# microsoft/tf2-gnn

Hardware: AMD Instinct MI355X
Metric: edges/sec (fwd+bwd) RGCN H=320 L=4, PPI-shaped batch, 1/2/4/8 MI355X (higher is better)
Workload: dtype f32; 1 GPU; rmat30k: V=30000 E=900000 per GPU (one batch per rank, replicas) edge_types=4 D=320 H=320 layers=4 RGCN (PPI_RGCN.json stack settings), step = edge bucketing of the next batch (2nd stream, overlapped) + forward (training mode) + f...

## Files before the change

### tf2_gnn_amd/csrc/graph.hip

```cpp
#include <algorithm>
#include <cstdlib>
#include <mutex>
#include <vector>

#include "common.hpp"
#include "graph.hpp"

namespace tfgnn {

static thread_local char g_err[512] = "";

void set_error(const char* fmt, ...) {
  va_list ap;
  va_start(ap, fmt);
  vsnprintf(g_err, sizeof(g_err), fmt, ap);
  va_end(ap);
}

static int64_t g_launch_counts[TFGNN_KFAM_COUNT] = {0};
void count_launch(int family) {
  if (family >= 0 && family < TFGNN_KFAM_COUNT) __atomic_fetch_add(&g_launch_counts[family], 1, __ATOMIC_RELAXED);
}

}
// ... 53 lines not shown
  for (int w = 0; w < (tid >> 6); ++w) wave_off += wave_tot[w];
  int32_t excl = wave_off + incl - sum;
#pragma unroll
  for (int i = 0; i < SCAN_ITEMS; ++i) {
    int64_t idx = base + i;
    if (idx < n) out[idx] = excl;
    excl += v[i];
  }
  if (tid == SCAN_THREADS - 1 && block_sums) block_sums[blockIdx.x] = wave_off + incl;
}

__global__ void __launch_bounds__(SCAN_THREADS)
scan_add_offsets_kernel(int32_t* __restrict__ out, const int32_t* __restrict__ block_offs, int64_t n) {
  const int32_t off = block_offs[blockIdx.x];
  const int64_t base = (int64_t)blockIdx.x * SCAN_TILE;
  for (int i = threadIdx.x; i < SCAN_TILE; i += SCAN_THREADS) {
    int64_t idx = base + i;
    if (idx < n) out[idx] += off;
  }
}

static size_t scan_scratch_elems(int64_t n) {
  size_t total = 0;
  while (n > SCAN_TILE) {
    n = ceil_div(n, SCAN_TILE);
    total += (size_t)n;
  }
  return total + 1;
}

static int exclusive_scan_i32(const int32_t* in, int32_t* out, int64_t n, int32_t* scratch,
                              hipStream_t s) {
  if (n <= 0) return TFGNN_OK;
  int64_t nb = ceil_div(n, SCAN_TILE);
  if (nb == 1) {
    hipLaunchKernelGGL(scan_tiles_kernel, dim3(1), dim3(SCAN_THREADS), 0, s, in, out, (int32_t*)nullptr, n);
    TFGNN_LAUNCH_CHECK();
    return TFGNN_OK;
  }
  hipLaunchKernelGGL(scan_tiles_kernel, dim3((unsigned)nb), dim3(SCAN_THREADS), 0, s, in, out, scratch, n);
  TFGNN_LAUNCH_CHECK();
  int rc = exclusive_scan_i32(scratch, scratch, nb, scratch + nb, s);
  if (rc) return rc;
  hipLaunchKernelGGL(scan_add_offsets_kernel, dim3((unsigned)nb), dim3(SCAN_THREADS), 0, s, out, scratch, n);
  TFGNN_LAUNCH_CHECK();
  return TFGNN_OK;
}

constexpr int EL_INLINE = 8;
struct EdgeLists {
  const int32_t* const* adj;
  const int64_t* edge_off;
  const int32_t* adj_v[EL_INLINE];
  int64_t off_v[EL_INLINE + 1];
  int L;
  int inline_tables;
};

__device__ __forceinline__ int find_type(const int64_t* __restrict__ edge_off, int L, int64_t g) {
  int lo = 0, hi = L;
  while (hi - lo > 1) {
    int mid = (lo + hi) >> 1;
    if (edge_off[mid] <= g) lo = mid; else hi = mid;
  }
  return lo;
}

__device__ __forceinline__ void load_edge(const EdgeLists& el, int64_t g, int64_t& src, int64_t& dst, int& l) {
  const int32_t* a;
  if (el.inline_tables) {
    l = 0;
#pragma unroll
    for (int i = 1; i < EL_INLINE; ++i) l += (i < el.L && el.off_v[i] <= g) ? 1 : 0;
    a = el.adj_v[l] + 2 * (g - el.off_v[l]);
  } else {
    l = find_type(el.edge_off, el.L, g);
    a = el.adj[l] + 2 * (g - el.edge_off[l]);
  }
  src = a[0];
  dst = a[1];
}

constexpr int RS_THREADS = 512;
constexpr int RS_ROUNDS = 16;
constexpr int RS_WAVES = RS_THREADS / 64;
constexpr int RS_WAVE_KEYS = 64 * RS_ROUNDS;
constexpr int RS_TILE = RS_THREADS * RS_ROUNDS;
constexpr int RS_DIGIT_BITS = 9;
constexpr int RS_RADIX = 1 << RS_DIGIT_BITS;
static_assert(RS_RADIX == RS_THREADS, "one digit per thread");

template <typename KeyT>
__global__ void __launch_bounds__(RS_THREADS)
fill_keys_kernel(EdgeLists el, int64_t E, int64_t V, int sec_bits, KeyT* __restrict__ comp_d, KeyT* __restrict__ comp_s,
                 int32_t* __restrict__ hist, int nblk_ld, int32_t* __restrict__ err_flag) {
  __shared__ int32_t h[2][RS_RADIX];
  const int tid = threadIdx.x;
  h[0][tid] = 0;
  h[1][tid] = 0;
  __syncthreads();
  const int64_t base = (int64_t)blockIdx.x * RS_TILE;
#pragma unroll 4
  for (int r = 0; r < RS_ROUNDS; ++r) {
    const int64_t g = base + r * RS_THREADS + tid;
    if (g < E) {
      int64_t src, dst;
      int l;
      load_edge(el, g, src, dst, l);
      if (src < 0 || src >= V || dst < 0 || dst >= V) {
        atomicOr(err_flag, 1);
        src = 0;
        dst = 0;
      }
      const KeyT kd = (KeyT)(((uint64_t)(dst * el.L + l) << sec_bits) | (uint64_t)src);
      const KeyT ks = (KeyT)(((uint64_t)(src * el.L + l) << sec_bits) | (uint64_t)dst);
      comp_d[g] = kd;
      comp_s[g] = ks;
      atomicAdd(&h[0][(int)((kd >> sec_bits) & (RS_RADIX - 1))], 1);
      atomicAdd(&h[1][(int)((ks >> sec_bits) & (RS_RADIX - 1))], 1);
    }
  }
  __syncthreads();
  hist[(int64_t)tid * nblk_ld + blockIdx.x] = h[0][tid];
  hist[(int64_t)(RS_RADIX + tid) * nblk_ld + blockIdx.x] = h[1][tid];
}

template <typename KeyT>
__global__ void __launch_bounds__(RS_THREADS)
rs_hist_kernel(const KeyT* __restrict__ comp_d, const KeyT* __restrict__ comp_s, int64_t n, int shift,
               int32_t* __restrict__ hist, int nblk_ld) {
  __shared__ int32_t h[RS_RADIX];
  const int tid = threadIdx.x;
  const int side = blockIdx.y;
  const KeyT* __restrict__ comp = side ? comp_s : comp_d;
  h[tid] = 0;
  __syncthreads();
  const int64_t base = (int64_t)blockIdx.x * RS_TILE;
#pragma unroll 4
  for (int r = 0; r < RS_ROUNDS; ++r) {
    const int64_t idx = base + r * RS_THREADS + tid;
    if (idx < n) atomicAdd(&h[(int)((comp[idx] >> shift) & (RS_RADIX - 1))], 1);
  }
  __syncthreads();
  hist[(int64_t)(side * RS_RADIX + tid) * nblk_ld + blockIdx.x] = h[tid];
}

template <typename KeyT, bool PAY>
__global__ void __launch_bounds__(RS_THREADS)
rs_scatter_kernel(const KeyT* __restrict__ in_d, const KeyT* __restrict__ in_s, const uint32_t* __restrict__ pin_d,
                  const uint32_t* __restrict__ pin_s, int64_t n, int shift, const int32_t* __restrict__ hist, int nblk,
                  int nblk_ld, KeyT* __restrict__ out_d, KeyT* __restrict__ out_s, uint32_t* __restrict__ pout_d,
                  uint32_t* __restrict__ pout_s) {
  __shared__ int32_t wbase[RS_WAVES][RS_RADIX];
  __shared__ int32_t wtot[RS_WAVES];
  const int tid = threadIdx.x;
  const int lane = tid & 63, wave = tid >> 6;
  const int side = blockIdx.y;
  const KeyT* __restrict__ kin = side ? in_s : in_d;
  const uint32_t* __restrict__ pin = side ? pin_s : pin_d;
  KeyT* __restrict__ kout = side ? out_s : out_d;
  uint32_t* __restrict__ pout = side ? pout_s : pout_d;
  volatile int32_t* mine_base = &wbase[wave][0];
#pragma unroll
  for (int i = 0; i < RS_RADIX / 64; ++i) mine_base[lane + 64 * i] = 0;
  __builtin_amdgcn_wave_barrier();
  const int64_t wave0 = (int64_t)blockIdx.x * RS_TILE + (int64_t)wave * RS_WAVE_KEYS;
  const unsigned long long lt_mask = lane == 0 ? 0ull : (~0ull >> (64 - lane));
  KeyT key[RS_ROUNDS];
  uint32_t pl[PAY ? RS_ROUNDS : 1];
  int32_t info[RS_ROUNDS];
#pragma unroll
  for (int r = 0; r < RS_ROUNDS; ++r) {
    const int64_t idx = wave0 + r * 64 + lane;
    const bool valid = idx < n;
    key[r] = valid ? kin[idx] : (KeyT)0;
    if (PAY) pl[r] = valid ? (pin ? pin[idx] : (uint32_t)idx) : 0u;
  }
#pragma unroll
  for (int r = 0; r < RS_ROUNDS; ++r) {
    const bool valid = wave0 + r * 64 + lane < n;
    const int d = (int)((key[r] >> shift) & (RS_RADIX - 1));
    unsigned long long peers = __ballot(valid);
#pragma unroll
    for (int b = 0; b < RS_DIGIT_BITS; ++b) {
      const unsigned long long m = __ballot((d >> b) & 1);
      peers &= ((d >> b) & 1) ? m : ~m;
    }
    const int rank = __popcll(peers & lt_mask);
    const int cnt = __popcll(peers);
    info[r] = valid ? (rank | (cnt << 8) | (1 << 16)) : 0;
    if (valid && rank == 0) mine_base[d] = mine_base[d] + cnt;
    __builtin_amdgcn_wave_barrier();
  }
  __syncthreads();
  int32_t tot = 0, before = 0;
  {
    const int32_t* __restrict__ row = hist + (int64_t)(side * RS_RADIX + tid) * nblk_ld;
    const int me = (int)blockIdx.x;
    for (int b0 = 0; b0 < nblk; b0 += 16) {
      int4 v[4];
#pragma unroll
      for (int u = 0; u < 4; ++u)
        v[u] = b0 + 4 * u < nblk ? *reinterpret_cast<const int4*>(row + b0 + 4 * u) : make_int4(0, 0, 0, 0);
#pragma unroll
      for (int u = 0; u < 4; ++u) {
        const int b = b0 + 4 * u;
        const int e[4] = {v[u].x, v[u].y, v[u].z, v[u].w};
#pragma unroll
        for (int k = 0; k < 4; ++k)
          if (b + k < nblk) {
            tot += e[k];
            if (b + k < me) before += e[k];
          }
      }
    }
  }
  int32_t incl = tot;
#pragma unroll
  for (int o = 1; o < 64; o <<= 1) {
    const int32_t t = __shfl_up(incl, o, 64);
    if (lane >= o) incl += t;
  }
  if (lane == 63) wtot[wave] = incl;
  __syncthreads();
  {
    int32_t off = 0;
    for (int w = 0; w < wave; ++w) off += wtot[w];
    int32_t running = off + incl - tot + before;
#pragma unroll
    for (int w = 0; w < RS_WAVES; ++w) {
      const int32_t c = wbase[w][tid];
      wbase[w][tid] = running;
      running += c;
    }
  }
  __syncthreads();
#pragma unroll
  for (int r = 0; r < RS_ROUNDS; ++r) {
    const bool valid = (info[r] >> 16) & 1;
    const int d = (int)((key[r] >> shift) & (RS_RADIX - 1));
    const int rank = info[r] & 255, cnt = (info[r] >> 8) & 255;
    const int32_t b = valid ? mine_base[d] : 0;
    __builtin_amdgcn_wave_barrier();
    if (valid && rank == 0) mine_base[d] = b + cnt;
    __builtin_amdgcn_wave_barrier();
    if (valid) {
      kout[b + rank] = key[r];
      if (PAY) pout[b + rank] = pl[r];
    }
  }
}

template <typename KeyT>
__global__ void rowptr_from_sorted_kernel(const KeyT* __restrict__ comp_d, const KeyT* __restrict__ comp_s, int64_t E,
                                          int sec_bits, int64_t R, int32_t* __restrict__ rowptr_d,
                                          int32_t* __restrict__ rowptr_s) {
  const KeyT* __restrict__ comp = blockIdx.y ? comp_s : comp_d;
  int32_t* __restrict__ rowptr = blockIdx.y ? rowptr_s : rowptr_d;
  for (int64_t r = (int64_t)blockIdx.x * blockDim.x + threadIdx.x; r <= R; r += (int64_t)gridDim.x * blockDim.x) {
    int64_t lo = 0, hi = E;
    while (lo < hi) {
      const int64_t mid = (lo + hi) >> 1;
      if ((int64_t)((uint64_t)comp[mid] >> sec_bits) < r) lo = mid + 1; else hi = mid;
    }
    rowptr[r] = (int32_t)lo;
  }
}

struct PlanJob {
  const int32_t* rowptr;
  int64_t R;
  int thr, chunk;
  int32_t* counters;
  int32_t *item_row, *item_chunk, *item_slot, *multi_row, *multi_base, *multi_n;
  int32_t *bin_count, *bin_cursor, *short_rows;
  int want_items;
};
struct PlanJobs {
  PlanJob j[2];
};

__device__ __forceinline__ void plan_rows_body(const int32_t* __restrict__ rowptr, int64_t R, int long_threshold, int chunk_edges,
                                 int32_t* __restrict__ counters,
                                 int32_t* __restrict__ item_row, int32_t* __restrict__ item_chunk,
                                 int32_t* __restrict__ item_slot, int32_t* __restrict__ multi_row,
                                 int32_t* __restrict__ multi_base, int32_t* __restrict__ multi_n) {
  for (int64_t r = (int64_t)blockIdx.x * blockDim.x + threadIdx.x; r < R; r += (int64_t)gridDim.x * blockDim.x) {
    const int32_t len = rowptr[r + 1] - rowptr[r];
    if (len <= long_threshold) continue;
    const int32_t n = (len + chunk_edges - 1) / chunk_edges;
    const int32_t base = atomicAdd(&counters[0], n);
    int32_t pb = -1;
    if (n > 1) {
      const int32_t m = atomicAdd(&counters[1], 1);
      pb = atomicAdd(&counters[2], n);
      multi_row[m] = (int32_t)r;
      multi_base[m] = pb;
      multi_n[m] = n;
// ... 58 lines not shown
      acc += bin_count[i];
    }
  }
  constexpr int TILE = 256 * SHORT_TILE_ROWS;
  for (int64_t tile = blockIdx.x; tile * TILE < R; tile += gridDim.x) {
    for (int i = threadIdx.x; i <= thr; i += 256) h[i] = 0;
    __syncthreads();
    int32_t len[SHORT_TILE_ROWS];
    int rank[SHORT_TILE_ROWS];
#pragma unroll
    for (int k = 0; k < SHORT_TILE_ROWS; ++k) {
      const int64_t r = tile * TILE + k * 256 + threadIdx.x;
      len[k] = r < R ? rowptr[r + 1] - rowptr[r] : -1;
      rank[k] = (len[k] >= 0 && len[k] <= thr) ? atomicAdd(&h[len[k]], 1) : 0;
    }
    __syncthreads();
    for (int i = threadIdx.x; i <= thr; i += 256)
      if (h[i]) base[i] = atomicAdd(&bin_cursor[i], h[i]);
    __syncthreads();
#pragma unroll
    for (int k = 0; k < SHORT_TILE_ROWS; ++k)
      if (len[k] >= 0 && len[k] <= thr)
        short_rows[start[len[k]] + base[len[k]] + rank[k]] = (int32_t)(tile * TILE + k * 256 + threadIdx.x);
    __syncthreads();
  }
}

__global__ void nz_flags_kernel(const int32_t* __restrict__ rowptr, int64_t V, int L, int32_t* __restrict__ flags,
                                int32_t* __restrict__ node_cnt) {
  const int64_t R = V * L;
  for (int64_t i = (int64_t)blockIdx.x * blockDim.x + threadIdx.x; i <= R; i += (int64_t)gridDim.x * blockDim.x) {
    if (i < R) {
      const int64_t l = i / V, v = i - l * V;
      const int64_t r = v * L + l;
      flags[i] = rowptr[r + 1] > rowptr[r] ? 1 : 0;
    } else {
      flags[i] = 0;
    }
    if (i <= V) {
      int32_t c = 0;
      if (i < V)
        for (int l = 0; l < L; ++l) c += rowptr[i * L + l + 1] > rowptr[i * L + l] ? 1 : 0;
      node_cnt[i] = c;
    }
  }
}

__global__ void nz_fill_kernel(const int32_t* __restrict__ rowptr, const int32_t* __restrict__ scan_t, int64_t V,
                               int L, int32_t* __restrict__ cpos, int32_t* __restrict__ nzrow,
                               int32_t* __restrict__ nz_node, int32_t* __restrict__ nz_off) {
  const int64_t R = V * L;
  for (int64_t i = (int64_t)blockIdx.x * blockDim.x + threadIdx.x; i < R; i += (int64_t)gridDim.x * blockDim.x) {
    const int64_t l = i / V, v = i - l * V;
    const int64_t r = v * L + l;
    const int32_t c = scan_t[i];
    if (rowptr[r + 1] > rowptr[r]) {
      cpos[r] = c;
      nzrow[c] = (int32_t)r;
      nz_node[c] = (int32_t)v;
    } else {
      cpos[r] = -1;
    }
    if (v == 0) nz_off[l] = c;
    if (i == R - 1) nz_off[L] = scan_t[R];
  }
}

__global__ void nz_cols_kernel(const int32_t* __restrict__ cpos, const int32_t* __restrict__ nodeptr_nz, int64_t V,
                               int L, int32_t* __restrict__ col_nz) {
  for (int64_t v = (int64_t)blockIdx.x * blockDim.x + threadIdx.x; v < V; v += (int64_t)gridDim.x * blockDim.x) {
    int32_t j = nodeptr_nz[v];
    for (int l = 0; l < L; ++l) {
      const int32_t c = cpos[v * L + l];
      if (c >= 0) col_nz[j++] = c;
    }
  }
}

__device__ __forceinline__ int node_pattern(const int32_t* __restrict__ rowptr, int64_t v, int L) {
  int m = 0;
  for (int l = 0; l < L; ++l) m |= (rowptr[v * L + l + 1] > rowptr[v * L + l]) ? (1 << l) : 0;
  return m;
}
__global__ void __launch_bounds__(256) pattern_count_kernel(const int32_t* __restrict__ rowptr, int64_t V, int L,
                                                            int32_t* __restrict__ bins ) {
  __shared__ int h[256];
  h[threadIdx.x] = 0;
  __syncthreads();
  for (int64_t v = (int64_t)blockIdx.x * 256 + threadIdx.x; v < V; v += (int64_t)gridDim.x * 256) atomicAdd(&h[node_pattern(rowptr, v, L)], 1);
  __syncthreads();
  if (h[threadIdx.x]) atomicAdd(&bins[threadIdx.x], h[threadIdx.x]);
}
__global__ void __launch_bounds__(256) pattern_place_kernel(const int32_t* __restrict__ rowptr, int64_t V, int L,
                                                            const int32_t* __restrict__ bins, int32_t* __restrict__ cursor ,
                                                            int32_t* __restrict__ pos, int32_t* __restrict__ node_at,
                                                            int32_t* __restrict__ rowmap) {
  __shared__ int base[256], h[256], slot0[256];
  {
    h[threadIdx.x] = bins[threadIdx.x];
    __syncthreads();
    const int key = ((8 - __popc((int)threadIdx.x)) << 8) | (int)threadIdx.x;
    int acc = 0;
    for (int m = 0; m < 256; ++m) acc += ((((8 - __popc(m)) << 8) | m) < key) ? h[m] : 0;
    base[threadIdx.x] = acc;
    __syncthreads();
  }
  for (int64_t v0 = (int64_t)blockIdx.x * 256; v0 < V; v0 += (int64_t)gridDim.x * 256) {
    h[threadIdx.x] = 0;
    __syncthreads();
    const int64_t v = v0 + threadIdx.x;
    int m = 0, rank = 0;
    if (v < V) {
      m = node_pattern(rowptr, v, L);
      rank = atomicAdd(&h[m], 1);
    }
    __syncthreads();
    if (h[threadIdx.x]) slot0[threadIdx.x] = atomicAdd(&cursor[threadIdx.x], h[threadIdx.x]);
    __syncthreads();
    if (v < V) {
      const int32_t p = base[m] + slot0[m] + rank;
      if (pos) pos[v] = p;
      node_at[p] = (int32_t)v;
      if (rowmap)
        for (int l = 0; l < L; ++l) rowmap[v * L + l] = p * L + l;
    }
    __syncthreads();
  }
}
__global__ void __launch_bounds__(128) pattern_tilemask_kernel(const int32_t* __restrict__ rowptr, const int32_t* __restrict__ node_at,
                                                               int64_t V, int L, uint8_t* __restrict__ tilemask) {
  __shared__ int m;
  if (threadIdx.x == 0) m = 0;
  __syncthreads();
  const int64_t p = (int64_t)blockIdx.x * 128 + threadIdx.x;
  if (p < V) atomicOr(&m, node_pattern(rowptr, node_at[p], L));
  __syncthreads();
  if (threadIdx.x == 0) tilemask[blockIdx.x] = (uint8_t)m;
}

template <typename KeyT, bool PAY>
__global__ void unpack_kernel(const KeyT* __restrict__ comp_d, const KeyT* __restrict__ comp_s, const uint32_t* __restrict__ pay_d,
                              const uint32_t* __restrict__ pay_s, int sec_bits, int64_t E, int L, int64_t R,
                              const int32_t* __restrict__ rowptr_d, const int32_t* __restrict__ rowptr_s,
                              int32_t* __restrict__ col_d, int32_t* __restrict__ eid_d, int32_t* __restrict__ coll_d,
                              float* __restrict__ invdeg_edge_d, int32_t* __restrict__ eid_to_pos, int32_t* __restrict__ row_node,
                              int32_t* __restrict__ col_s, int32_t* __restrict__ eid_s, int32_t* __restrict__ coll_s,
                              float* __restrict__ invdeg_edge_s, float* __restrict__ invdeg_d, int32_t* __restrict__ nodeptr_d,
                              int32_t* __restrict__ nodeptr_s, int first_job) {
  const int job = (int)blockIdx.y + first_job;
  if (job == 2) {
    for (int64_t r = (int64_t)blockIdx.x * blockDim.x + threadIdx.x; r <= R; r += (int64_t)gridDim.x * blockDim.x) {
      if (r < R) {
        const int32_t len = rowptr_d[r + 1] - rowptr_d[r];
        invdeg_d[r] = len > 0 ? 1.0f / ((float)len + kSmallNumber) : 0.f;
      }
      if (r % L == 0) {
        nodeptr_d[r / L] = rowptr_d[r];
        nodeptr_s[r / L] = rowptr_s[r];
      }
    }
    return;
  }
  const int by_src = job;
  const KeyT* __restrict__ comp = by_src ? comp_s : comp_d;
  const uint32_t* __restrict__ pay = by_src ? pay_s : pay_d;
  int32_t* __restrict__ col = by_src ? col_s : col_d;
  int32_t* __restrict__ eid = by_src ? eid_s : eid_d;
  int32_t* __restrict__ coll = by_src ? coll_s : coll_d;
  float* __restrict__ invdeg_edge = by_src ? invdeg_edge_s : invdeg_edge_d;
  const uint64_t sec_mask = ((uint64_t)1 << sec_bits) - 1;
  for (int64_t p = (int64_t)blockIdx.x * blockDim.x + threadIdx.x; p < E; p += (int64_t)gridDim.x * blockDim.x) {
    const uint64_t c = (uint64_t)comp[p];
    const int32_t other = (int32_t)(c & sec_mask);
    const int32_t row = (int32_t)(c >> sec_bits);
    const int l = row % L;
    col[p] = other;
    if (PAY) eid[p] = (int32_t)pay[p];
    const int64_t cl = (int64_t)other * L + l;
    coll[p] = (int32_t)cl;
    const int64_t trow = by_src ? cl : (int64_t)row;
    const int32_t len = rowptr_d[trow + 1] - rowptr_d[trow];
    invdeg_edge[p] = len > 0 ? 1.0f / ((float)len + kSmallNumber) : 0.f;
    if (!by_src) {
      row_node[p] = row / L;
      if (PAY) eid_to_pos[pay[p]] = (int32_t)p;
    }
  }
}

__global__ void src2dst_kernel(const int32_t* __restrict__ eid_s, const int32_t* __restrict__ eid_to_pos_d,
                               int64_t E, int32_t* __restrict__ src2dst, int32_t* __restrict__ dst2src) {
  for (int64_t p = (int64_t)blockIdx.x * blockDim.x + threadIdx.x; p < E;
       p += (int64_t)gridDim.x * blockDim.x) {
    const int32_t q = eid_to_pos_d[eid_s[p]];
    src2dst[p] = q;
    dst2src[q] = (int32_t)p;
  }
}

}


namespace tfgnn {
struct PoolEntry {
  void* ptr;
  size_t bytes;
  hipEvent_t ready;
};
static std::mutex g_pool_mutex;
static std::vector<PoolEntry> g_dev_pool, g_pinned_pool;
constexpr size_t POOL_MAX_ENTRIES = 12;

static void* pool_take(std::vector<PoolEntry>& pool, size_t bytes, size_t* got, hipStream_t s) {
  std::lock_guard<std::mutex> lock(g_pool_mutex);
// ... 39 lines not shown
  (void)hipFree(p);
}
static hipError_t pinned_alloc(void** p, size_t bytes, size_t* got) {
  if (bytes < 4096) bytes = 4096;
  *p = pool_take(g_pinned_pool, bytes, got, nullptr);
  if (*p) return hipSuccess;
  *got = bytes;
  return hipHostMalloc(p, bytes, hipHostMallocDefault);
}
static void pinned_release(void* p, size_t bytes) {
  if (!p) return;
  {
    std::lock_guard<std::mutex> lock(g_pool_mutex);
    if (g_pinned_pool.size() < POOL_MAX_ENTRIES) {
      g_pinned_pool.push_back({p, bytes, nullptr});
      return;
    }
  }
  (void)hipHostFree(p);
}
}

namespace {
struct SlabPlan {
  size_t total = 0;
  size_t take(size_t bytes) {
    size_t off = total;
    total += (bytes + 255) & ~(size_t)255;
    return off;
  }
};
}

static void graph_release_all(tfgnn_graph* g, hipStream_t last_use = nullptr, bool in_use = false) {
  using namespace tfgnn;
  if (!g) return;
  if (g->event) (void)hipEventDestroy((hipEvent_t)g->event);
  dev_release(g->scratch, g->scratch_bytes, last_use, in_use);
  dev_release(g->slab, g->slab_bytes, last_use, in_use);
  pinned_release(g->pinned, g->pinned_bytes);
  delete g;
}

namespace {
using namespace tfgnn;

constexpr unsigned kPartsAll = TFGNN_GRAPH_PART_PLAN_TYPED | TFGNN_GRAPH_PART_PLAN_NODE | TFGNN_GRAPH_PART_COMPACT |
                               TFGNN_GRAPH_PART_EDGE_MAPS | TFGNN_GRAPH_PART_EDGE_IDS | TFGNN_GRAPH_PART_DST_PATTERN;

void view_plan_parameters(int view_long[4], int view_chunk[4]) {
  const int dl[4] = {LONG_ROW_THRESHOLD_TYPED, LONG_ROW_THRESHOLD, LONG_ROW_THRESHOLD_TYPED, LONG_ROW_THRESHOLD};
  const int dc[4] = {ITEM_CHUNK_TYPED, ITEM_CHUNK, ITEM_CHUNK_TYPED, ITEM_CHUNK};
  for (int v = 0; v < 4; ++v) {
    view_long[v] = dl[v];
    view_chunk[v] = dc[v];
    if (view_long[v] > SHORT_BINS - 1) view_long[v] = SHORT_BINS - 1;
    if (view_chunk[v] < view_long[v]) view_chunk[v] = view_long[v];
  }
}

unsigned blocks_for(int64_t n) { return (unsigned)std::max<int64_t>(1, std::min<int64_t>(ceil_div(n, 256), 8192)); }

int build_plans(tfgnn_graph* g, int node_views, int32_t* counters, int32_t* bins, hipStream_t s) {
  PlanJobs jobs{};
  int64_t max_rows = 0;
  for (int k = 0; k < 2; ++k) {
    const int v = 2 * k + node_views;
    CsrPlan& pl = g->views[v].plan;
    PlanJob& j = jobs.j[k];
    j.rowptr = g->views[v].rowptr;
    j.R = g->views[v].num_rows;
    j.thr = pl.long_threshold;
    j.chunk = pl.item_chunk_edges;
    j.counters = counters + 16 + 4 * v;
    j.item_row = pl.item_row; j.item_chunk = pl.item_chunk; j.item_slot = pl.item_slot;
    j.multi_row = pl.multi_row; j.multi_base = pl.multi_base; j.multi_n = pl.multi_n;
    j.bin_count = bins + (size_t)v * 2 * SHORT_BINS;
    j.bin_cursor = j.bin_count + SHORT_BINS;
    j.short_rows = pl.short_rows;
    j.want_items = g->E > 0;
    max_rows = std::max(max_rows, j.R);
  }
  if (max_rows <= 0) return TFGNN_OK;
  hipLaunchKernelGGL(plan_hist_kernel, dim3(blocks_for(max_rows), 4), dim3(256), 0, s, jobs);
  TFGNN_LAUNCH_CHECK();
  const unsigned scat_blocks = (unsigned)std::min<int64_t>(ceil_div(max_rows, 256 * SHORT_TILE_ROWS), 4096);
  hipLaunchKernelGGL(short_scatter_kernel, dim3(scat_blocks, 2), dim3(256), 0, s, jobs);
  TFGNN_LAUNCH_CHECK();
  return TFGNN_OK;
}

size_t compact_scratch_bytes(int64_t R, int64_t V) {
  return (size_t)(R + 2) * 4 + 256 + (scan_scratch_elems(R + 1) + scan_scratch_elems(V + 1)) * 4 + 64;
}

int build_compact(tfgnn_graph* g, char* scratch, hipStream_t s) {
  const int L = g->L;
  const int64_t V = g->V, R = g->R;
  int32_t* flags = (int32_t*)scratch;
  int32_t* scan_tmp = (int32_t*)(scratch + (((size_t)(R + 2) * 4 + 255) & ~(size_t)255));
  for (int side = 0; side < 2; ++side) {
    CompactBuckets& cb = g->compact[side];
    const int32_t* rp = side == 0 ? g->rowptr_d : g->rowptr_s;
    if (L > 0) {
      hipLaunchKernelGGL(nz_flags_kernel, dim3(blocks_for(R + 1)), dim3(256), 0, s, rp, V, L, flags, cb.nodeptr_nz);
      int rc = exclusive_scan_i32(flags, flags, R + 1, scan_tmp, s);
      if (rc) return rc;
      rc = exclusive_scan_i32(cb.nodeptr_nz, cb.nodeptr_nz, V + 1, scan_tmp, s);
      if (rc) return rc;
      if (R > 0) {
        hipLaunchKernelGGL(nz_fill_kernel, dim3(blocks_for(R)), dim3(256), 0, s, rp, flags, V, L, cb.cpos, cb.nzrow,
                           cb.nz_node, cb.nz_off);
        hipLaunchKernelGGL(nz_cols_kernel, dim3(blocks_for(V)), dim3(256), 0, s, cb.cpos, cb.nodeptr_nz, V, L, cb.col_nz);
      } else {
        TFGNN_HIP_CHECK(hipMemsetAsync(cb.nz_off, 0, (size_t)(L + 1) * 4, s));
      }
    } else {
      TFGNN_HIP_CHECK(hipMemsetAsync(cb.nz_off, 0, (size_t)(L + 1) * 4, s));
      TFGNN_HIP_CHECK(hipMemsetAsync(cb.nodeptr_nz, 0, (V + 1) * 4, s));
    }
    TFGNN_HIP_CHECK(hipMemcpyAsync((char*)g->pinned + 256 + (size_t)(L + 1) * 16 + (size_t)side * (L + 1) * 4, cb.nz_off,
                                   (size_t)(L + 1) * 4, hipMemcpyDeviceToHost, s));
  }
  TFGNN_LAUNCH_CHECK();
  return TFGNN_OK;
}

int build_dst_pattern(tfgnn_graph* g, int32_t* pat, hipStream_t s) {
  if (g->V <= 0 || g->L <= 0 || g->L > 8) return TFGNN_OK;
  const unsigned blocks = (unsigned)std::min<int64_t>(ceil_div(g->V, 256), 1024);
  hipLaunchKernelGGL(pattern_count_kernel, dim3(blocks), dim3(256), 0, s, (const int32_t*)g->rowptr_d, g->V, g->L, pat);
  hipLaunchKernelGGL(pattern_place_kernel, dim3(blocks), dim3(256), 0, s, (const int32_t*)g->rowptr_d, g->V, g->L, (const int32_t*)pat,
                     pat + 256, g->pat_pos_d, g->pat_node_d, g->pat_rowmap_d);
  hipLaunchKernelGGL(pattern_tilemask_kernel, dim3((unsigned)ceil_div(g->V, 128)), dim3(128), 0, s, (const int32_t*)g->rowptr_d,
                     (const int32_t*)g->pat_node_d, g->V, g->L, g->pat_tilemask_d);
  int32_t* pat_s = pat + 512;
  hipLaunchKernelGGL(pattern_count_kernel, dim3(blocks), dim3(256), 0, s, (const int32_t*)g->rowptr_s, g->V, g->L, pat_s);
  hipLaunchKernelGGL(pattern_place_kernel, dim3(blocks), dim3(256), 0, s, (const int32_t*)g->rowptr_s, g->V, g->L, (const int32_t*)pat_s,
                     pat_s + 256, (int32_t*)nullptr, g->pat_node_s, (int32_t*)nullptr);
  hipLaunchKernelGGL(pattern_tilemask_kernel, dim3((unsigned)ceil_div(g->V, 128)), dim3(128), 0, s, (const int32_t*)g->rowptr_s,
                     (const int32_t*)g->pat_node_s, g->V, g->L, g->pat_tilemask_s);
  TFGNN_LAUNCH_CHECK();
  return TFGNN_OK;
}

int build_edge_maps(tfgnn_graph* g, hipStream_t s) {
  if (g->E > 0) {
    hipLaunchKernelGGL(src2dst_kernel, dim3(blocks_for(g->E)), dim3(256), 0, s, g->eid_s, g->eid2pos, g->E, g->src2dst, g->dst2src);
    TFGNN_LAUNCH_CHECK();
  }
  return TFGNN_OK;
}

template <typename KeyT, bool PAY>
int build_core(tfgnn_graph* g, const EdgeLists& el, char* keys, char* pays, int32_t* hist, int nblk, int nblk_ld,
               int32_t* counters, hipStream_t s) {
  const int64_t E = g->E, R = g->R, V = g->V;
  const int L = g->L;
  const int sec_bits = g->sec_bits, total_bits = g->total_bits;
  KeyT* kbuf[2][2];
  uint32_t* pbuf[2][2];
  for (int side = 0; side < 2; ++side)
    for (int b = 0; b < 2; ++b) {
      kbuf[side][b] = (KeyT*)(keys + (size_t)(side * 2 + b) * (size_t)E * 8);
      pbuf[side][b] = PAY ? (uint32_t*)(pays + (size_t)(side * 2 + b) * (size_t)E * 4) : nullptr;
    }
  hipLaunchKernelGGL((fill_keys_kernel<KeyT>), dim3(nblk), dim3(RS_THREADS), 0, s, el, E, V, sec_bits, kbuf[0][0], kbuf[1][0],
                     hist, nblk_ld, counters + 2);
  int cur = 0;
  bool first = true;
  for (int shift = sec_bits; shift < total_bits; shift += RS_DIGIT_BITS) {
    if (!first)
      hipLaunchKernelGGL((rs_hist_kernel<KeyT>), dim3(nblk, 2), dim3(RS_THREADS), 0, s, (const KeyT*)kbuf[0][cur],
                         (const KeyT*)kbuf[1][cur], E, shift, hist, nblk_ld);
    hipLaunchKernelGGL((rs_scatter_kernel<KeyT, PAY>), dim3(nblk, 2), dim3(RS_THREADS), 0, s, (const KeyT*)kbuf[0][cur],
                       (const KeyT*)kbuf[1][cur], first ? (const uint32_t*)nullptr : (const uint32_t*)pbuf[0][cur],
                       first ? (const uint32_t*)nullptr : (const uint32_t*)pbuf[1][cur], E, shift, (const int32_t*)hist, nblk, nblk_ld,
                       kbuf[0][cur ^ 1], kbuf[1][cur ^ 1], pbuf[0][cur ^ 1], pbuf[1][cur ^ 1]);
    cur ^= 1;
    first = false;
  }
  hipLaunchKernelGGL((rowptr_from_sorted_kernel<KeyT>), dim3(blocks_for(R + 1), 2), dim3(256), 0, s, (const KeyT*)kbuf[0][cur],
                     (const KeyT*)kbuf[1][cur], E, sec_bits, R, g->rowptr_d, g->rowptr_s);
  hipLaunchKernelGGL((unpack_kernel<KeyT, PAY>), dim3(blocks_for(std::max(E, R + 1)), 3), dim3(256), 0, s, (const KeyT*)kbuf[0][cur],
                     (const KeyT*)kbuf[1][cur], (const uint32_t*)pbuf[0][cur], (const uint32_t*)pbuf[1][cur], sec_bits, E, L, R,
                     (const int32_t*)g->rowptr_d, (const int32_t*)g->rowptr_s, g->col_d, g->eid_d, g->coll_d, g->invdeg_edge_d,
                     g->eid2pos, g->tgt_d, g->col_s, g->eid_s, g->coll_s, g->invdeg_edge_s, g->invdeg_d, g->nodeptr_d,
                     g->nodeptr_s, 0);
  TFGNN_LAUNCH_CHECK();
  return TFGNN_OK;
}

struct CoreScratch {
  size_t keys, pays, hist, counters, ptrs, off, total;
  int nblk, nblk_ld;
};
CoreScratch core_scratch(int64_t E, int L, bool pay) {
  CoreScratch c{};
  SlabPlan tmp;
  c.nblk = (int)ceil_div(E > 0 ? E : 1, RS_TILE);
  c.nblk_ld = (c.nblk + 3) & ~3;
  c.keys = tmp.take((size_t)E * 8 * 4);
  c.pays = tmp.take(pay ? (size_t)E * 4 * 4 : 0);
  c.hist = tmp.take((size_t)2 * RS_RADIX * c.nblk_ld * 4 + 16);
  c.counters = tmp.take((size_t)(64 + 4 * 2 * SHORT_BINS + 1024) * 4);
  c.ptrs = tmp.take((size_t)(L + 1) * 8);
  c.off = tmp.take((size_t)(L + 1) * 8);
  c.total = tmp.total;
  return c;
}

int run_core(tfgnn_graph* g, bool pay, char* scratch, const CoreScratch& cs, hipStream_t s) {
  const int L = g->L;
  EdgeLists el{};
  el.L = L;
  el.inline_tables = L <= EL_INLINE;
  if (el.inline_tables) {
    for (int l = 0; l < EL_INLINE; ++l) el.adj_v[l] = l < L ? g->h_adj[l] : nullptr;
    for (int l = 0; l <= EL_INLINE; ++l) el.off_v[l] = l <= L ? g->h_off[l] : g->E;
  } else {
    const int32_t** d_ptrs = (const int32_t**)(scratch + cs.ptrs);
    int64_t* d_off = (int64_t*)(scratch + cs.off);
    char* hp = (char*)g->pinned + 256;
    const int32_t** h_ptrs = (const int32_t**)hp;
    int64_t* h_off = (int64_t*)(hp + (size_t)(L + 1) * 8);
    for (int l = 0; l < L; ++l) h_ptrs[l] = g->h_adj[l];
    for (int l = 0; l <= L; ++l) h_off[l] = g->h_off[l];
    TFGNN_HIP_CHECK(hipMemcpyAsync(d_ptrs, h_ptrs, (size_t)L * 8, hipMemcpyHostToDevice, s));
    TFGNN_HIP_CHECK(hipMemcpyAsync(d_off, h_off, (size_t)(L + 1) * 8, hipMemcpyHostToDevice, s));
    el.adj = d_ptrs;
    el.edge_off = d_off;
  }
  char* keys = scratch + cs.keys;
  char* pays = scratch + cs.pays;
  int32_t* hist = (int32_t*)(scratch + cs.hist);
  int32_t* counters = (int32_t*)(scratch + cs.counters);
  if (g->total_bits <= 32)
    return pay ? build_core<uint32_t, true>(g, el, keys, pays, hist, cs.nblk, cs.nblk_ld, counters, s)
               : build_core<uint32_t, false>(g, el, keys, pays, hist, cs.nblk, cs.nblk_ld, counters, s);
  return pay ? build_core<uint64_t, true>(g, el, keys, pays, hist, cs.nblk, cs.nblk_ld, counters, s)
             : build_core<uint64_t, false>(g, el, keys, pays, hist, cs.nblk, cs.nblk_ld, counters, s);
}
}

static int graph_create_impl(int num_edge_types, int64_t num_nodes, const int32_t* const* d_adjacency,
                             const int64_t* num_edges, unsigned parts, void* stream, tfgnn_graph** out_graph) {
  using namespace tfgnn;
  TFGNN_REQUIRE(out_graph != nullptr, "out_graph is NULL");
  *out_graph = nullptr;
  TFGNN_REQUIRE(num_edge_types >= 0 && num_nodes >= 0, "negative sizes");
  TFGNN_REQUIRE(num_edge_types == 0 || (d_adjacency && num_edges), "adjacency arrays are NULL");
  TFGNN_REQUIRE((parts & ~kPartsAll) == 0, "unknown graph part bits 0x%x", parts);
  hipStream_t s = (hipStream_t)stream;
  (void)dropout_epoch_word();
  const int L = num_edge_types;
  const int64_t V = num_nodes;
  std::vector<int64_t> edge_off(L + 1, 0);
  for (int l = 0; l < L; ++l) {
    TFGNN_REQUIRE(num_edges[l] >= 0, "num_edges[%d] < 0", l);
    TFGNN_REQUIRE(num_edges[l] == 0 || d_adjacency[l] != nullptr, "adjacency list %d is NULL", l);
    edge_off[l + 1] = edge_off[l] + num_edges[l];
  }
  const int64_t E = edge_off[L];
  const int64_t R = V * (int64_t)L;
  TFGNN_REQUIRE(R < ((int64_t)1 << 31) - 1 && E < ((int64_t)1 << 31) - 1,
                "graph too large for int32 indexing (V*L=%lld, E=%lld)", (long long)R, (long long)E);
  TFGNN_REQUIRE(L <= 256, "at most 256 edge types are supported (got %d)", L);

  tfgnn_graph* g = new tfgnn_graph();
  g->L = L;
  g->V = V;
  g->E = E;
  g->R = R;

  SlabPlan plan;
  const size_t o_rowptr_d = plan.take((R + 1) * 4), o_rowptr_s = plan.take((R + 1) * 4);
  const size_t o_col_d = plan.take(E * 4), o_eid_d = plan.take(E * 4), o_coll_d = plan.take(E * 4);
  const size_t o_col_s = plan.take(E * 4), o_eid_s = plan.take(E * 4), o_coll_s = plan.take(E * 4);
  const size_t o_nodeptr_d = plan.take((V + 1) * 4), o_nodeptr_s = plan.take((V + 1) * 4);
  const size_t o_src2dst = plan.take(E * 4), o_dst2src = plan.take(E * 4);
  const size_t o_tgt_d = plan.take(E * 4), o_eid2pos = plan.take(E * 4);
  const size_t o_pat_pos = plan.take((V + 1) * 4), o_pat_node = plan.take((V + 1) * 4), o_pat_rowmap = plan.take((R + 1) * 4);
  const size_t o_pat_mask = plan.take((size_t)ceil_div(V > 0 ? V : 1, 128) + 16);
  const size_t o_pat_node_s = plan.take((V + 1) * 4), o_pat_mask_s = plan.take((size_t)ceil_div(V > 0 ? V : 1, 128) + 16);
  const size_t o_invdeg_d = plan.take((R + 1) * 4);
  const size_t o_invdeg_es = plan.take(E * 4), o_invdeg_ed = plan.take(E * 4);
  size_t o_cb[2][6];
  for (int side = 0; side < 2; ++side) {
    o_cb[side][0] = plan.take((R + 1) * 4);
    o_cb[side][1] = plan.take((R + 1) * 4);
    o_cb[side][2] = plan.take((R + 1) * 4);
    o_cb[side][3] = plan.take((size_t)(L + 1) * 4);
    o_cb[side][4] = plan.take((V + 1) * 4);
    o_cb[side][5] = plan.take((R + 1) * 4);
  }
  int view_long[4], view_chunk[4];
  view_plan_parameters(view_long, view_chunk);
  const int min_long = std::min(std::min(view_long[0], view_long[1]), std::min(view_long[2], view_long[3]));
  const int min_chunk = std::min(std::min(view_chunk[0], view_chunk[1]), std::min(view_chunk[2], view_chunk[3]));
  const size_t max_items = (size_t)(E / min_long + 1), max_multi = (size_t)(E / min_chunk + 1);
  size_t o_item[4][3], o_multi[4][3];
  for (int v = 0; v < 4; ++v) {
    for (int k = 0; k < 3; ++k) o_item[v][k] = plan.take(max_items * 4);
    for (int k = 0; k < 3; ++k) o_multi[v][k] = plan.take(max_multi * 4);
  }
  size_t o_short[4];
  for (int v = 0; v < 4; ++v) o_short[v] = plan.take((size_t)((v & 1) ? V : R) * 4 + 4);
  const size_t persistent = plan.total;
  if (parts & TFGNN_GRAPH_PART_EDGE_MAPS) parts |= TFGNN_GRAPH_PART_EDGE_IDS;
  const bool with_ids = (parts & TFGNN_GRAPH_PART_EDGE_IDS) != 0;
  const CoreScratch cs = core_scratch(E, L, with_ids);
  const size_t t_compact = (cs.total + 255) & ~(size_t)255;
  const size_t scratch_total = t_compact + ((parts & TFGNN_GRAPH_PART_COMPACT) ? compact_scratch_bytes(R, V) : 0);
  g->h_adj.assign(d_adjacency, d_adjacency + L);
  g->h_off = edge_off;
  {
    int sec_bits = 1;
    while (((int64_t)1 << sec_bits) < V) ++sec_bits;
    int row_bits = 1;
    while (((int64_t)1 << row_bits) < (R > 0 ? R : 1)) ++row_bits;
    g->sec_bits = sec_bits;
    g->total_bits = sec_bits + row_bits;
  }

// ... 411 lines not shown
```

Before: 376.4 million edges/s.

## Add a separate tile-scan pass to radix sort and batch pattern kernels across sides

The radix sort now runs a dedicated scan kernel over the per-tile histograms, which are stored in tile-major layout. Each scatter block reads its precomputed exclusive offset and the digit total instead of scanning every tile's histogram itself. The tile size is cut from 16 to 4 rounds so more blocks run in parallel. The dst/src pattern kernels are merged into single launches using gridDim.y=2, and the plan histogram grid is capped. The cost is one extra launch per digit pass and four times as many tiles, so the histogram buffers grow.

```diff
diff --git a/tf2_gnn_amd/csrc/graph.hip b/tf2_gnn_amd/csrc/graph.hip
--- a/tf2_gnn_amd/csrc/graph.hip
+++ b/tf2_gnn_amd/csrc/graph.hip
@@ -159,7 +159,7 @@
 }
 
 constexpr int RS_THREADS = 512;
-constexpr int RS_ROUNDS = 16;
+constexpr int RS_ROUNDS = 4;
 constexpr int RS_WAVES = RS_THREADS / 64;
 constexpr int RS_WAVE_KEYS = 64 * RS_ROUNDS;
 constexpr int RS_TILE = RS_THREADS * RS_ROUNDS;
@@ -170,14 +170,14 @@
 template <typename KeyT>
 __global__ void __launch_bounds__(RS_THREADS)
 fill_keys_kernel(EdgeLists el, int64_t E, int64_t V, int sec_bits, KeyT* __restrict__ comp_d, KeyT* __restrict__ comp_s,
-                 int32_t* __restrict__ hist, int nblk_ld, int32_t* __restrict__ err_flag) {
+                 int32_t* __restrict__ hist, int nblk, int32_t* __restrict__ err_flag) {
   __shared__ int32_t h[2][RS_RADIX];
   const int tid = threadIdx.x;
   h[0][tid] = 0;
   h[1][tid] = 0;
   __syncthreads();
   const int64_t base = (int64_t)blockIdx.x * RS_TILE;
-#pragma unroll 4
+#pragma unroll
   for (int r = 0; r < RS_ROUNDS; ++r) {
     const int64_t g = base + r * RS_THREADS + tid;
     if (g < E) {
@@ -198,14 +198,14 @@
     }
   }
   __syncthreads();
-  hist[(int64_t)tid * nblk_ld + blockIdx.x] = h[0][tid];
-  hist[(int64_t)(RS_RADIX + tid) * nblk_ld + blockIdx.x] = h[1][tid];
+  hist[(int64_t)blockIdx.x * RS_RADIX + tid] = h[0][tid];
+  hist[((int64_t)nblk + blockIdx.x) * RS_RADIX + tid] = h[1][tid];
 }
 
 template <typename KeyT>
 __global__ void __launch_bounds__(RS_THREADS)
 rs_hist_kernel(const KeyT* __restrict__ comp_d, const KeyT* __restrict__ comp_s, int64_t n, int shift,
-               int32_t* __restrict__ hist, int nblk_ld) {
+               int32_t* __restrict__ hist, int nblk) {
   __shared__ int32_t h[RS_RADIX];
   const int tid = threadIdx.x;
   const int side = blockIdx.y;
@@ -213,20 +213,56 @@
   h[tid] = 0;
   __syncthreads();
   const int64_t base = (int64_t)blockIdx.x * RS_TILE;
-#pragma unroll 4
+#pragma unroll
   for (int r = 0; r < RS_ROUNDS; ++r) {
     const int64_t idx = base + r * RS_THREADS + tid;
     if (idx < n) atomicAdd(&h[(int)((comp[idx] >> shift) & (RS_RADIX - 1))], 1);
   }
   __syncthreads();
-  hist[(int64_t)(side * RS_RADIX + tid) * nblk_ld + blockIdx.x] = h[tid];
+  hist[((int64_t)side * nblk + blockIdx.x) * RS_RADIX + tid] = h[tid];
+}
+
+constexpr int TS_DIGITS = 32, TS_SEGS = 32, TS_BATCH = 8;
+static_assert(RS_RADIX % TS_DIGITS == 0, "whole workgroups");
+__global__ void __launch_bounds__(TS_DIGITS * TS_SEGS)
+rs_tile_scan_kernel(int32_t* __restrict__ hist, int32_t* __restrict__ totals, int nblk) {
+  __shared__ int32_t seg_sum[TS_SEGS][TS_DIGITS];
+  const int dx = threadIdx.x % TS_DIGITS, seg = threadIdx.x / TS_DIGITS;
+  const int side = blockIdx.y;
+  const int d = blockIdx.x * TS_DIGITS + dx;
+  const int per = (nblk + TS_SEGS - 1) / TS_SEGS;
+  const int t0 = min(seg * per, nblk), t1 = min(t0 + per, nblk);
+  int32_t* col = hist + (int64_t)side * nblk * RS_RADIX + d;
+  int32_t sum = 0;
+  for (int t = t0; t < t1; t += TS_BATCH) {
+    int32_t v[TS_BATCH];
+#pragma unroll
+    for (int k = 0; k < TS_BATCH; ++k) v[k] = t + k < t1 ? col[(int64_t)(t + k) * RS_RADIX] : 0;
+#pragma unroll
+    for (int k = 0; k < TS_BATCH; ++k) sum += v[k];
+  }
+  seg_sum[seg][dx] = sum;
+  __syncthreads();
+  int32_t acc = 0;
+  for (int q = 0; q < seg; ++q) acc += seg_sum[q][dx];
+  for (int t = t0; t < t1; t += TS_BATCH) {
+    int32_t v[TS_BATCH];
+#pragma unroll
+    for (int k = 0; k < TS_BATCH; ++k) v[k] = t + k < t1 ? col[(int64_t)(t + k) * RS_RADIX] : 0;
+#pragma unroll
+    for (int k = 0; k < TS_BATCH; ++k) {
+      if (t + k < t1) col[(int64_t)(t + k) * RS_RADIX] = acc;
+      acc += v[k];
+    }
+  }
+  if (seg == TS_SEGS - 1) totals[side * RS_RADIX + d] = acc;
 }
 
 template <typename KeyT, bool PAY>
 __global__ void __launch_bounds__(RS_THREADS)
 rs_scatter_kernel(const KeyT* __restrict__ in_d, const KeyT* __restrict__ in_s, const uint32_t* __restrict__ pin_d,
-                  const uint32_t* __restrict__ pin_s, int64_t n, int shift, const int32_t* __restrict__ hist, int nblk,
-                  int nblk_ld, KeyT* __restrict__ out_d, KeyT* __restrict__ out_s, uint32_t* __restrict__ pout_d,
+                  const uint32_t* __restrict__ pin_s, int64_t n, int shift, const int32_t* __restrict__ hist,
+                  const int32_t* __restrict__ totals, int nblk, KeyT* __restrict__ out_d, KeyT* __restrict__ out_s, uint32_t* __restrict__ pout_d,
                   uint32_t* __restrict__ pout_s) {
   __shared__ int32_t wbase[RS_WAVES][RS_RADIX];
   __shared__ int32_t wtot[RS_WAVES];
@@ -238,6 +274,8 @@
   KeyT* __restrict__ kout = side ? out_s : out_d;
   uint32_t* __restrict__ pout = side ? pout_s : pout_d;
   volatile int32_t* mine_base = &wbase[wave][0];
+  const int32_t before = hist[((int64_t)side * nblk + blockIdx.x) * RS_RADIX + tid];
+  const int32_t tot = totals[side * RS_RADIX + tid];
 #pragma unroll
   for (int i = 0; i < RS_RADIX / 64; ++i) mine_base[lane + 64 * i] = 0;
   __builtin_amdgcn_wave_barrier();
@@ -268,29 +306,6 @@
     info[r] = valid ? (rank | (cnt << 8) | (1 << 16)) : 0;
     if (valid && rank == 0) mine_base[d] = mine_base[d] + cnt;
     __builtin_amdgcn_wave_barrier();
-  }
-  __syncthreads();
-  int32_t tot = 0, before = 0;
-  {
-    const int32_t* __restrict__ row = hist + (int64_t)(side * RS_RADIX + tid) * nblk_ld;
-    const int me = (int)blockIdx.x;
-    for (int b0 = 0; b0 < nblk; b0 += 16) {
-      int4 v[4];
-#pragma unroll
-      for (int u = 0; u < 4; ++u)
-        v[u] = b0 + 4 * u < nblk ? *reinterpret_cast<const int4*>(row + b0 + 4 * u) : make_int4(0, 0, 0, 0);
-#pragma unroll
-      for (int u = 0; u < 4; ++u) {
-        const int b = b0 + 4 * u;
-        const int e[4] = {v[u].x, v[u].y, v[u].z, v[u].w};
-#pragma unroll
-        for (int k = 0; k < 4; ++k)
-          if (b + k < nblk) {
-            tot += e[k];
-            if (b + k < me) before += e[k];
-          }
-      }
-    }
   }
   int32_t incl = tot;
 #pragma unroll
@@ -515,20 +530,30 @@
   for (int l = 0; l < L; ++l) m |= (rowptr[v * L + l + 1] > rowptr[v * L + l]) ? (1 << l) : 0;
   return m;
 }
-__global__ void __launch_bounds__(256) pattern_count_kernel(const int32_t* __restrict__ rowptr, int64_t V, int L,
-                                                            int32_t* __restrict__ bins ) {
+struct PatternSides {
+  const int32_t* rowptr[2];
+  int32_t* bins[2];
+  int32_t *pos[2], *node_at[2], *rowmap[2];
+  uint8_t* tilemask[2];
+};
+__global__ void __launch_bounds__(256) pattern_count_kernel(PatternSides ps, int64_t V, int L) {
   __shared__ int h[256];
+  const int32_t* __restrict__ rowptr = ps.rowptr[blockIdx.y];
+  int32_t* __restrict__ bins = ps.bins[blockIdx.y];
   h[threadIdx.x] = 0;
   __syncthreads();
   for (int64_t v = (int64_t)blockIdx.x * 256 + threadIdx.x; v < V; v += (int64_t)gridDim.x * 256) atomicAdd(&h[node_pattern(rowptr, v, L)], 1);
   __syncthreads();
   if (h[threadIdx.x]) atomicAdd(&bins[threadIdx.x], h[threadIdx.x]);
 }
-__global__ void __launch_bounds__(256) pattern_place_kernel(const int32_t* __restrict__ rowptr, int64_t V, int L,
-                                                            const int32_t* __restrict__ bins, int32_t* __restrict__ cursor ,
-                                                            int32_t* __restrict__ pos, int32_t* __restrict__ node_at,
-                                                            int32_t* __restrict__ rowmap) {
+__global__ void __launch_bounds__(256) pattern_place_kernel(PatternSides ps, int64_t V, int L) {
   __shared__ int base[256], h[256], slot0[256];
+  const int32_t* __restrict__ rowptr = ps.rowptr[blockIdx.y];
+  const int32_t* __restrict__ bins = ps.bins[blockIdx.y];
+  int32_t* __restrict__ cursor = ps.bins[blockIdx.y] + 256;
+  int32_t* __restrict__ pos = ps.pos[blockIdx.y];
+  int32_t* __restrict__ node_at = ps.node_at[blockIdx.y];
+  int32_t* __restrict__ rowmap = ps.rowmap[blockIdx.y];
   {
     h[threadIdx.x] = bins[threadIdx.x];
     __syncthreads();
@@ -560,9 +585,11 @@
     __syncthreads();
   }
 }
-__global__ void __launch_bounds__(128) pattern_tilemask_kernel(const int32_t* __restrict__ rowptr, const int32_t* __restrict__ node_at,
-                                                               int64_t V, int L, uint8_t* __restrict__ tilemask) {
+__global__ void __launch_bounds__(128) pattern_tilemask_kernel(PatternSides ps, int64_t V, int L) {
   __shared__ int m;
+  const int32_t* __restrict__ rowptr = ps.rowptr[blockIdx.y];
+  const int32_t* __restrict__ node_at = ps.node_at[blockIdx.y];
+  uint8_t* __restrict__ tilemask = ps.tilemask[blockIdx.y];
   if (threadIdx.x == 0) m = 0;
   __syncthreads();
   const int64_t p = (int64_t)blockIdx.x * 128 + threadIdx.x;
@@ -768,7 +795,8 @@
     max_rows = std::max(max_rows, j.R);
   }
   if (max_rows <= 0) return TFGNN_OK;
-  hipLaunchKernelGGL(plan_hist_kernel, dim3(blocks_for(max_rows), 4), dim3(256), 0, s, jobs);
+  const unsigned hist_blocks = (unsigned)std::max<int64_t>(1, std::min<int64_t>(ceil_div(max_rows, 1024), 1024));
+  hipLaunchKernelGGL(plan_hist_kernel, dim3(hist_blocks, 4), dim3(256), 0, s, jobs);
   TFGNN_LAUNCH_CHECK();
   const unsigned scat_blocks = (unsigned)std::min<int64_t>(ceil_div(max_rows, 256 * SHORT_TILE_ROWS), 4096);
   hipLaunchKernelGGL(short_scatter_kernel, dim3(scat_blocks, 2), dim3(256), 0, s, jobs);
@@ -814,18 +842,17 @@
 
 int build_dst_pattern(tfgnn_graph* g, int32_t* pat, hipStream_t s) {
   if (g->V <= 0 || g->L <= 0 || g->L > 8) return TFGNN_OK;
+  PatternSides ps{};
+  ps.rowptr[0] = g->rowptr_d;           ps.rowptr[1] = g->rowptr_s;
+  ps.bins[0] = pat;                     ps.bins[1] = pat + 512;
+  ps.pos[0] = g->pat_pos_d;             ps.pos[1] = nullptr;
+  ps.node_at[0] = g->pat_node_d;        ps.node_at[1] = g->pat_node_s;
+  ps.rowmap[0] = g->pat_rowmap_d;       ps.rowmap[1] = nullptr;
+  ps.tilemask[0] = g->pat_tilemask_d;   ps.tilemask[1] = g->pat_tilemask_s;
   const unsigned blocks = (unsigned)std::min<int64_t>(ceil_div(g->V, 256), 1024);
-  hipLaunchKernelGGL(pattern_count_kernel, dim3(blocks), dim3(256), 0, s, (const int32_t*)g->rowptr_d, g->V, g->L, pat);
-  hipLaunchKernelGGL(pattern_place_kernel, dim3(blocks), dim3(256), 0, s, (const int32_t*)g->rowptr_d, g->V, g->L, (const int32_t*)pat,
-                     pat + 256, g->pat_pos_d, g->pat_node_d, g->pat_rowmap_d);
-  hipLaunchKernelGGL(pattern_tilemask_kernel, dim3((unsigned)ceil_div(g->V, 128)), dim3(128), 0, s, (const int32_t*)g->rowptr_d,
-                     (const int32_t*)g->pat_node_d, g->V, g->L, g->pat_tilemask_d);
-  int32_t* pat_s = pat + 512;
-  hipLaunchKernelGGL(pattern_count_kernel, dim3(blocks), dim3(256), 0, s, (const int32_t*)g->rowptr_s, g->V, g->L, pat_s);
-  hipLaunchKernelGGL(pattern_place_kernel, dim3(blocks), dim3(256), 0, s, (const int32_t*)g->rowptr_s, g->V, g->L, (const int32_t*)pat_s,
-                     pat_s + 256, (int32_t*)nullptr, g->pat_node_s, (int32_t*)nullptr);
-  hipLaunchKernelGGL(pattern_tilemask_kernel, dim3((unsigned)ceil_div(g->V, 128)), dim3(128), 0, s, (const int32_t*)g->rowptr_s,
-                     (const int32_t*)g->pat_node_s, g->V, g->L, g->pat_tilemask_s);
+  hipLaunchKernelGGL(pattern_count_kernel, dim3(blocks, 2), dim3(256), 0, s, ps, g->V, g->L);
+  hipLaunchKernelGGL(pattern_place_kernel, dim3(blocks, 2), dim3(256), 0, s, ps, g->V, g->L);
+  hipLaunchKernelGGL(pattern_tilemask_kernel, dim3((unsigned)ceil_div(g->V, 128), 2), dim3(128), 0, s, ps, g->V, g->L);
   TFGNN_LAUNCH_CHECK();
   return TFGNN_OK;
 }
@@ -839,8 +866,8 @@
 }
 
 template <typename KeyT, bool PAY>
-int build_core(tfgnn_graph* g, const EdgeLists& el, char* keys, char* pays, int32_t* hist, int nblk, int nblk_ld,
-               int32_t* counters, hipStream_t s) {
+int build_core(tfgnn_graph* g, const EdgeLists& el, char* keys, char* pays, int32_t* hist, int nblk, int32_t* counters,
+               hipStream_t s) {
   const int64_t E = g->E, R = g->R, V = g->V;
   const int L = g->L;
   const int sec_bits = g->sec_bits, total_bits = g->total_bits;
@@ -852,16 +879,19 @@
       pbuf[side][b] = PAY ? (uint32_t*)(pays + (size_t)(side * 2 + b) * (size_t)E * 4) : nullptr;
     }
   hipLaunchKernelGGL((fill_keys_kernel<KeyT>), dim3(nblk), dim3(RS_THREADS), 0, s, el, E, V, sec_bits, kbuf[0][0], kbuf[1][0],
-                     hist, nblk_ld, counters + 2);
+                     hist, nblk, counters + 2);
+  int32_t* totals = hist + (size_t)2 * nblk * RS_RADIX;
   int cur = 0;
   bool first = true;
   for (int shift = sec_bits; shift < total_bits; shift += RS_DIGIT_BITS) {
     if (!first)
       hipLaunchKernelGGL((rs_hist_kernel<KeyT>), dim3(nblk, 2), dim3(RS_THREADS), 0, s, (const KeyT*)kbuf[0][cur],
-                         (const KeyT*)kbuf[1][cur], E, shift, hist, nblk_ld);
+                         (const KeyT*)kbuf[1][cur], E, shift, hist, nblk);
+    hipLaunchKernelGGL(rs_tile_scan_kernel, dim3(RS_RADIX / TS_DIGITS, 2), dim3(TS_DIGITS * TS_SEGS), 0, s, hist, totals, nblk);
     hipLaunchKernelGGL((rs_scatter_kernel<KeyT, PAY>), dim3(nblk, 2), dim3(RS_THREADS), 0, s, (const KeyT*)kbuf[0][cur],
                        (const KeyT*)kbuf[1][cur], first ? (const uint32_t*)nullptr : (const uint32_t*)pbuf[0][cur],
-                       first ? (const uint32_t*)nullptr : (const uint32_t*)pbuf[1][cur], E, shift, (const int32_t*)hist, nblk, nblk_ld,
+                       first ? (const uint32_t*)nullptr : (const uint32_t*)pbuf[1][cur], E, shift, (const int32_t*)hist,
+                       (const int32_t*)totals, nblk,
                        kbuf[0][cur ^ 1], kbuf[1][cur ^ 1], pbuf[0][cur ^ 1], pbuf[1][cur ^ 1]);
     cur ^= 1;
     first = false;
@@ -879,16 +909,15 @@
 
 struct CoreScratch {
   size_t keys, pays, hist, counters, ptrs, off, total;
-  int nblk, nblk_ld;
+  int nblk;
 };
 CoreScratch core_scratch(int64_t E, int L, bool pay) {
   CoreScratch c{};
   SlabPlan tmp;
   c.nblk = (int)ceil_div(E > 0 ? E : 1, RS_TILE);
-  c.nblk_ld = (c.nblk + 3) & ~3;
   c.keys = tmp.take((size_t)E * 8 * 4);
   c.pays = tmp.take(pay ? (size_t)E * 4 * 4 : 0);
-  c.hist = tmp.take((size_t)2 * RS_RADIX * c.nblk_ld * 4 + 16);
+  c.hist = tmp.take((size_t)2 * RS_RADIX * ((size_t)c.nblk + 1) * 4);
   c.counters = tmp.take((size_t)(64 + 4 * 2 * SHORT_BINS + 1024) * 4);
   c.ptrs = tmp.take((size_t)(L + 1) * 8);
   c.off = tmp.take((size_t)(L + 1) * 8);
@@ -922,10 +951,10 @@
   int32_t* hist = (int32_t*)(scratch + cs.hist);
   int32_t* counters = (int32_t*)(scratch + cs.counters);
   if (g->total_bits <= 32)
-    return pay ? build_core<uint32_t, true>(g, el, keys, pays, hist, cs.nblk, cs.nblk_ld, counters, s)
-               : build_core<uint32_t, false>(g, el, keys, pays, hist, cs.nblk, cs.nblk_ld, counters, s);
-  return pay ? build_core<uint64_t, true>(g, el, keys, pays, hist, cs.nblk, cs.nblk_ld, counters, s)
-             : build_core<uint64_t, false>(g, el, keys, pays, hist, cs.nblk, cs.nblk_ld, counters, s);
+    return pay ? build_core<uint32_t, true>(g, el, keys, pays, hist, cs.nblk, counters, s)
+               : build_core<uint32_t, false>(g, el, keys, pays, hist, cs.nblk, counters, s);
+  return pay ? build_core<uint64_t, true>(g, el, keys, pays, hist, cs.nblk, counters, s)
+             : build_core<uint64_t, false>(g, el, keys, pays, hist, cs.nblk, counters, s);
 }
 }
 
```

After: 377.6 million edges/s (median of 6 runs). No clear change (+0.3%).
